# mllam/neural-lam

Measured on AMD Instinct MI355X. Metric: training sample-steps/s (on_after_batch_transfer+fwd+wmse+bwd+allreduce+AdamW), GraphCast-LAM, MEPS-shaped grid, higher is better.
Workload: dtype f32; 1 GPU; cfg2: graph_lam, grid 238x268 (63784 nodes), 17 state vars, hidden_dim 64, 4 processor layers, ar_steps 1, batch 1/GPU, g2m/m2m/m2g edges 79236/57616/255136; global_batch=1, parallelism=dp1

## Files before the change

### include/nlam_hip.h

```cpp
#ifndef NLAM_HIP_H
#define NLAM_HIP_H

#include <stdint.h>

#ifdef __cplusplus
extern "C" {
#endif

#define NLAM_ABI_VERSION 8
#define NLAM_MAX_SRC 3
#define NLAM_MAX_CAT 6

#define NLAM_EINVAL (-1)
#define NLAM_EUNSUP (-2)

#define NLAM_F_ADD_SRC0   1u
#define NLAM_F_ADD_SRC1   2u
#define NLAM_F_MEAN       4u
#define NLAM_F_SILU_B     8u
#define NLAM_F_PRE_ADD   16u
#define NLAM_F_LEAF_WGRAD 32u
#define NLAM_F_WPACK_READY 64u
#define NLAM_F_NO_ACT 128u
#define NLAM_F_STORE_BF16 (1u << 10)
// ... 190 lines not shown
int64_t nlam_mlp_bwd_gemm_workspace_floats(const nlam_mlp_bwd_t* p);
int32_t nlam_mlp_bwd_gemm_blocks(const nlam_mlp_bwd_t* p);
int32_t nlam_mlp_fwd_gemm(const nlam_mlp_fwd_t* p, void* hip_stream);
int32_t nlam_mlp_bwd_gemm(const nlam_mlp_bwd_t* p, void* hip_stream);

typedef struct {
    const float* W1;
    const float* W2;
    float* fwd_image;
    float* bwd_image;
    int32_t hid, dout, nsrc;
    int32_t ldw1;
    int32_t width[NLAM_MAX_SRC];
    uint32_t flags;
} nlam_pack_job_t;
int64_t nlam_mlp_pack_floats(const nlam_pack_job_t* job, int32_t which);
typedef struct {
    unsigned char bytes[64];
} nlam_pack_rec_t;
int32_t nlam_mlp_fwd_pack_records(const nlam_mlp_fwd_t* p, nlam_pack_rec_t* out, int32_t cap, int32_t* kind);
int32_t nlam_mlp_bwd_pack_records(const nlam_mlp_bwd_t* p, nlam_pack_rec_t* out, int32_t cap, int32_t* kind);
int32_t nlam_pack_records(const nlam_pack_rec_t* recs_device, int32_t n, int32_t kind, void* hip_stream);
int32_t nlam_mlp_pack(const nlam_pack_job_t* jobs_device, int32_t njobs, void* hip_stream);

#define NLAM_MAX_GROUP 8
int32_t nlam_mlp_group_blocks(const int64_t* tiles, int32_t n, int32_t* blocks);
int32_t nlam_mlp_fwd_group(const nlam_mlp_fwd_t* ps, int32_t n, void* hip_stream);
int32_t nlam_mlp_bwd_group(const nlam_mlp_bwd_t* ps, int32_t n, void* hip_stream);
int32_t nlam_mlp_fwd_family(const nlam_mlp_fwd_t* p);
int32_t nlam_mlp_bwd_family(const nlam_mlp_bwd_t* p);
int32_t nlam_mlp_bwd_group_blocks(const nlam_mlp_bwd_t* ps, int32_t n, int32_t* blocks);
int32_t nlam_wgrad(const nlam_wgrad_t* p, void* hip_stream);
int32_t nlam_wgrad_group(const nlam_wgrad_t* ps, int32_t n, void* hip_stream);

int32_t nlam_segment_sum_groups(int64_t in_bstride, int32_t nseg, int32_t width);
int32_t nlam_segment_sum(const float* in, int64_t in_bstride, const int32_t* ptr, const int32_t* order,
                         const float* scale, float* out, int32_t nseg, int32_t width, int32_t batch,
                         void* hip_stream);
int32_t nlam_segment_sum_acc(const float* in, int64_t in_bstride, const int32_t* ptr, const int32_t* order,
                         const float* scale, float* out, int32_t nseg, int32_t width, int32_t batch,
                         void* hip_stream);
int32_t nlam_segment_sum_add(const float* in, int64_t in_bstride, const int32_t* ptr, const int32_t* order, const float* scale,
                             const float* extra, float* out, int32_t nseg, int32_t width, int32_t batch, void* hip_stream);

int32_t nlam_segment_sum_bf16(const uint16_t* in, int64_t in_bstride, const int32_t* ptr, const int32_t* order,
                              const float* scale, float* out, int32_t nseg, int32_t width, int32_t batch, void* hip_stream);

int32_t nlam_split_combine(float* buf, int64_t bstride, const int32_t* ptr, const int32_t* src, const int32_t* dst, int32_t n,
                           int32_t width, int32_t batch, void* hip_stream);

int32_t nlam_reduce_partials(const float* partials, int32_t nparts, int64_t stride, int32_t n, float* out,
                             int32_t accumulate, void* hip_stream);

#define NLAM_MAX_REDUCE_JOBS 40
typedef struct {
    const float* partials;
    float* out;
    int64_t stride;
    int32_t nparts;
    int32_t n;
    int32_t accumulate;
    int32_t ncols;
    int32_t ld;
    int32_t _pad;
} nlam_reduce_job_t;
typedef struct {
// ... 410 lines not shown
```

### neural_lam_amd/_lib.py

```python
from __future__ import annotations

import ctypes as C
import os
from pathlib import Path

HERE = Path(__file__).resolve().parent
LIB_PATH = Path(os.environ["NLAM_LIB"]) if os.environ.get("NLAM_LIB") else HERE / "libnlam_hip.so"

NLAM_MAX_SRC = 3
NLAM_MAX_CAT = 6
NLAM_MAX_REDUCE_JOBS = 40
NLAM_MAX_GROUP = 8
F_ADD_SRC0, F_ADD_SRC1, F_MEAN, F_SILU_B, F_PRE_ADD, F_LEAF_WGRAD, F_WPACK_READY, F_NO_ACT = 1, 2, 4, 8, 16, 32, 64, 128
F_STORE_BF16, F_A_BF16, F_S_BF16 = 1 << 10, 1 << 10, 1 << 11
F_ACC_DSRC0 = 1 << 12
F_WGRAD_SOLO = 1 << 13
TUNE_WBF_MIN_SUPERTILES = 1
TUNE_WGRAD_CHUNKS = 2
TUNE_LIN_WGS = 3
TUNE_WGRAD_MIN_PARTS = 4
TUNE_WGRAD_BIG_MIN_ROWS = 5
TUNE_WBF_HALF = 6
TUNE_LIN_GEMM = 7
TUNE_WBF_V4 = 8
# ... 84 lines not shown
    "nlam_mlp_bwd",
    "nlam_mlp_fwd_gemm_workspace_floats",
    "nlam_mlp_bwd_gemm_workspace_floats",
    "nlam_mlp_bwd_gemm_blocks",
    "nlam_mlp_fwd_gemm",
    "nlam_mlp_bwd_gemm",
    "nlam_mlp_pack_floats",
    "nlam_mlp_pack",
    "nlam_mlp_fwd_pack_records",
    "nlam_mlp_bwd_pack_records",
    "nlam_pack_records",
    "nlam_wgrad",
    "nlam_segment_sum",
    "nlam_segment_sum_acc",
    "nlam_segment_sum_add",
    "nlam_split_combine",
    "nlam_segment_sum_bf16",
    "nlam_store_bf16_supported",
    "nlam_reduce_partials",
    "nlam_reduce_jobs",
    "nlam_reduce_jobs_waves",
    "nlam_wmse_fwd",
    "nlam_wmse_bwd",
    "nlam_adamw_step",
    "nlam_adamw_step_resident",
    "nlam_standardize",
    "nlam_mlp_group_blocks",
    "nlam_mlp_fwd_group",
    "nlam_mlp_bwd_group",
    "nlam_mlp_fwd_family",
    "nlam_mlp_bwd_family",
    "nlam_mlp_bwd_group_blocks",
    "nlam_wgrad_group",
    "nlam_linear",
    "nlam_linear_plan",
    "nlam_segment_sum_groups",
    "nlam_pre_add_supported",
    "nlam_step_tail_fwd",
    "nlam_step_tail_bwd",
    "nlam_loss_fwd",
    "nlam_loss_bwd",
    "nlam_step_tail_loss_fwd",
    "nlam_step_tail_loss_bwd",
    "nlam_step_tail_ext_fwd",
    "nlam_step_tail_ext_bwd",
    "nlam_eval_metrics",
    "nlam_eval_workspace_floats",
    "nlam_concat",
    "nlam_window_len",
    "nlam_window_batch",
    "nlam_window_batch_ens",
    "nlam_window_moments",
    "nlam_moments_workspace_doubles",
    "nlam_grad_sumsq_workspace_doubles",
    "nlam_grad_sumsq",
    "nlam_adamw_step_controlled",
    "nlam_accum_begin",
    "nlam_adamw_step_accum",
    "nlam_adamw_step_resident_ema",
    "nlam_adamw_step_controlled_ema",
    "nlam_flat_swap",
    "nlam_forecast_init",
    "nlam_forecast_head",
    "nlam_forecast_tail",
    "nlam_forecast_finish",
    "nlam_forecast_workspace_floats",
# ... 672 lines not shown
    lib.nlam_window_moments.restype = i32
    lib.nlam_moments_workspace_doubles.argtypes = [i32, i32, i64, i32]
    lib.nlam_moments_workspace_doubles.restype = i64
    lib.nlam_grad_sumsq_workspace_doubles.argtypes = [i64]
    lib.nlam_grad_sumsq_workspace_doubles.restype = i64
    lib.nlam_grad_sumsq.argtypes = [vp, i64, vp, i64, f32, vp, vp]
    lib.nlam_grad_sumsq.restype = i32
    lib.nlam_adamw_step_controlled.argtypes = [C.POINTER(OptCtl), vp]
    lib.nlam_adamw_step_controlled.restype = i32
    lib.nlam_accum_begin.argtypes = [vp, i64, vp, vp]
    lib.nlam_accum_begin.restype = i32
    lib.nlam_adamw_step_accum.argtypes = [C.POINTER(OptCtl), C.POINTER(Accum), vp]
    lib.nlam_adamw_step_accum.restype = i32
    lib.nlam_adamw_step_resident_ema.argtypes = [vp, vp, vp, vp, i64, f32, f32, f32, f32, f32, vp, vp, f32, vp, C.POINTER(Ema)]
    lib.nlam_adamw_step_resident_ema.restype = i32
    lib.nlam_adamw_step_controlled_ema.argtypes = [C.POINTER(OptCtl), C.POINTER(Accum), C.POINTER(Ema), vp]
    lib.nlam_adamw_step_controlled_ema.restype = i32
    lib.nlam_flat_swap.argtypes = [vp, vp, i64, vp]
    lib.nlam_flat_swap.restype = i32
    lib.nlam_mlp_group_blocks.argtypes = [C.POINTER(C.c_int64), i32, C.POINTER(C.c_int32)]
    lib.nlam_mlp_group_blocks.restype = i32
    lib.nlam_mlp_fwd_group.argtypes = [C.POINTER(MlpFwd), i32, vp]
    lib.nlam_mlp_fwd_group.restype = i32
    lib.nlam_mlp_bwd_group.argtypes = [C.POINTER(MlpBwd), i32, vp]
    lib.nlam_mlp_bwd_group.restype = i32
    lib.nlam_mlp_fwd_family.argtypes = [C.POINTER(MlpFwd)]
    lib.nlam_mlp_fwd_family.restype = i32
    lib.nlam_mlp_bwd_family.argtypes = [C.POINTER(MlpBwd)]
    lib.nlam_mlp_bwd_family.restype = i32
    lib.nlam_mlp_bwd_group_blocks.argtypes = [C.POINTER(MlpBwd), i32, C.POINTER(i32)]
    lib.nlam_mlp_bwd_group_blocks.restype = i32
    lib.nlam_wgrad_group.argtypes = [C.POINTER(Wgrad), i32, vp]
    lib.nlam_wgrad_group.restype = i32
    lib.nlam_pre_add_supported.argtypes = [C.POINTER(MlpFwd)]
    lib.nlam_pre_add_supported.restype = i32
    lib.nlam_linear.argtypes = [C.POINTER(Linear), vp]
    lib.nlam_linear.restype = i32
    lib.nlam_linear_plan.argtypes = [C.POINTER(Linear)]
    lib.nlam_linear_plan.restype = i32
    lib.nlam_segment_sum_groups.argtypes = [i64, i32, i32]
    lib.nlam_segment_sum_groups.restype = i32
    lib.nlam_standardize.argtypes = [C.POINTER(StdJobs), vp]
    lib.nlam_standardize.restype = i32
    if lib.nlam_abi_version() != ABI_VERSION:
        raise RuntimeError("libnlam_hip.so ABI version mismatch")
    if os.environ.get("NLAM_LIN_WGS"):
        lib.nlam_set_tuning(TUNE_LIN_WGS, int(os.environ["NLAM_LIN_WGS"]))
    if os.environ.get("NLAM_WGRAD_BIG_MIN_ROWS"):
        lib.nlam_set_tuning(TUNE_WGRAD_BIG_MIN_ROWS, int(os.environ["NLAM_WGRAD_BIG_MIN_ROWS"]))
    if os.environ.get("NLAM_WGRAD_MIN_PARTS"):
        lib.nlam_set_tuning(TUNE_WGRAD_MIN_PARTS, int(os.environ["NLAM_WGRAD_MIN_PARTS"]))
    if os.environ.get("NLAM_WBF_HALF"):
        check(lib.nlam_set_tuning(TUNE_WBF_HALF, int(os.environ["NLAM_WBF_HALF"])), "nlam_set_tuning(NLAM_WBF_HALF)")
    if os.environ.get("NLAM_WBF_V4"):
        lib.nlam_set_tuning(TUNE_WBF_V4, int(os.environ["NLAM_WBF_V4"]))
    if os.environ.get("NLAM_LIN_GEMM"):
        lib.nlam_set_tuning(TUNE_LIN_GEMM, int(os.environ["NLAM_LIN_GEMM"]))
    if os.environ.get("NLAM_WGRAD_LDMA"):
        check(lib.nlam_set_tuning(TUNE_WGRAD_LDMA, int(os.environ["NLAM_WGRAD_LDMA"])), "nlam_set_tuning(NLAM_WGRAD_LDMA)")
    if os.environ.get("NLAM_WBF_EDGE"):
        check(lib.nlam_set_tuning(TUNE_WBF_EDGE, int(os.environ["NLAM_WBF_EDGE"])), "nlam_set_tuning(NLAM_WBF_EDGE)")
    if os.environ.get("NLAM_WGRAD_LDMA_VAR"):
        check(lib.nlam_set_tuning(TUNE_WGRAD_LDMA_VAR, int(os.environ["NLAM_WGRAD_LDMA_VAR"])), "nlam_set_tuning(NLAM_WGRAD_LDMA_VAR)")
    if os.environ.get("NLAM_WGRAD_DMA_R"):
        check(lib.nlam_set_tuning(TUNE_WGRAD_DMA_R, int(os.environ["NLAM_WGRAD_DMA_R"])), "nlam_set_tuning(NLAM_WGRAD_DMA_R)")
    if os.environ.get("NLAM_CHAIN_CUS"):
# ... 75 lines not shown
```

### neural_lam_amd/csrc/nlam_hip.hip

```cpp

#include <hip/hip_runtime.h>
#include <stdint.h>
#include <type_traits>

#include "../../include/nlam_hip.h"
#include <dlfcn.h>
#include <stdlib.h>
#include <string.h>

#ifndef NLAM_TU
#define NLAM_TU 0
#endif
#ifndef NLAM_RES_PRE
#define NLAM_RES_PRE 3
#endif
#ifndef NLAM_BWD_G_BATCH
#define NLAM_BWD_G_BATCH 2
#endif
#ifndef NLAM_LW_PREFETCH_X
#define NLAM_LW_PREFETCH_X 1
#endif
#ifndef NLAM_BWD_Z_EARLY
#define NLAM_BWD_Z_EARLY 1
#endif
#ifndef NLAM_BWD_R_EARLY
#define NLAM_BWD_R_EARLY 0
#endif
#ifndef NLAM_LIN_SK
#define NLAM_LIN_SK 4
#endif
#define NLAM_IN_TU(k) (NLAM_TU == 0 || NLAM_TU == (k))

namespace nlam_detail {
int32_t fwd_narrow(const nlam_mlp_fwd_t* p, hipStream_t stream);
int32_t bwd_narrow(const nlam_mlp_bwd_t* p, hipStream_t stream);
int32_t wgrad_narrow(const nlam_wgrad_t* p, int plan, hipStream_t stream);
int32_t fwd_wide(const nlam_mlp_fwd_t* p, int plan, hipStream_t stream);
int32_t bwd_wide(const nlam_mlp_bwd_t* p, int plan, hipStream_t stream);
int32_t fwd_wide_group(const nlam_mlp_fwd_t* ps, int n, hipStream_t stream);
int32_t bwd_wide_group(const nlam_mlp_bwd_t* ps, int n, hipStream_t stream);
int32_t fwd_check(const nlam_mlp_fwd_t* p);
int32_t bwd_check(const nlam_mlp_bwd_t* p);
int32_t wgrad_wide(const nlam_wgrad_t* p, hipStream_t stream);
int32_t fwd_wbf(const nlam_mlp_fwd_t* p, int plan, hipStream_t stream);
int32_t bwd_wbf(const nlam_mlp_bwd_t* p, int plan, hipStream_t stream);
int32_t wgrad_wbf(const nlam_wgrad_t* p, int plan, hipStream_t stream);
int32_t wgrad_wbf_group(const nlam_wgrad_t* ps, int n, hipStream_t stream);
extern int wbf_min_supertiles;
extern int wbf_half;
extern int wbf_v4;
extern int wgrad_chunks_per_wg;
extern int wgrad_ldma;
extern int chain_cus;
extern int wgrad_max_wgs;
extern int wbf_edge;
extern int wgrad_ldma_var;
extern int wgrad_dma_r;
extern int wgrad_min_parts;
extern int wgrad_min_parts_wide;
extern int wgrad_big_min_rows;
extern int lin_resident_wgs;
extern int lin_gemm;
extern long lin_gemm_big_rows;
}

typedef float f32x4 __attribute__((ext_vector_type(4)));
typedef float f32x16 __attribute__((ext_vector_type(16)));

#define MFMA32(a, b, c) __builtin_amdgcn_mfma_f32_32x32x2f32((a), (b), (c), 0, 0, 0)
// ... 2214 lines not shown
                p.vec_partials[((size_t)wg_id * kVecRows + 4 + wave) * p.vec_stride + lane] = s;
            }
        }
    }
}

template <int HB, int OB, int NS, bool RO = false>
__global__ __launch_bounds__(kBlockThreads) void mlp_bwd_fast_kernel(const nlam_mlp_bwd_t p) {
    mlp_bwd_fast_body<HB, OB, NS, false, kWavesPerBlock, RO>(p, xcd_slot((int)blockIdx.x, (int)gridDim.x), (int)gridDim.x);
}

struct bwd_group_t {
    nlam_mlp_bwd_t g[NLAM_MAX_GROUP];
    int n;
    int first[NLAM_MAX_GROUP + 1];
};

constexpr int kLeafWaves = 4;
template <int HB, int OB, int NS, bool LW>
__global__ __launch_bounds__(LW ? kLeafWaves * 64 : kBlockThreads) void mlp_bwd_fast_group_kernel(const bwd_group_t G) {
    int gi = 0;
#pragma unroll
    for (int k = 1; k < NLAM_MAX_GROUP; ++k)
        if (k < G.n && (int)blockIdx.x >= G.first[k]) gi = k;
    mlp_bwd_fast_body<HB, OB, NS, LW, LW ? kLeafWaves : kWavesPerBlock>(G.g[gi], (int)blockIdx.x - G.first[gi], G.first[gi + 1] - G.first[gi]);
}

constexpr int kWgradThreads = 256;
constexpr int kWgradRows = 32;
constexpr int kWgTile = kWgradRows * 64;


template <int NBW, bool SILU, int NS, int R>
__global__ __launch_bounds__(kWgradThreads) void wgrad_dma_kernel(const nlam_wgrad_t p) {
    static_assert(NS >= 0 && NS <= NLAM_MAX_SRC && R >= 1 && (NS > 0 || R == 1), "run-time source count: one chunk per interval");
    constexpr int MS = NS > 0 ? NS : NLAM_MAX_SRC;
    extern __shared__ __attribute__((aligned(16))) float smem[];
    const int nsrc = NS > 0 ? NS : p.nsrc;
    const int ntile = 1 + nsrc;
    const int lane = threadIdx.x & 63;
    const int wave = __builtin_amdgcn_readfirstlane(threadIdx.x >> 6);
    const int i = lane & 31, hi = lane >> 5;
    const int MB = (p.m + 31) >> 5;

    int blk_mb[NBW], blk_tile[NBW], blk_nb[NBW], blk_col0[NBW], blk_w[NBW];
    {
        int nb_total = 0;
#pragma unroll
        for (int s = 0; s < MS; ++s)
            if (s < nsrc) nb_total += (p.src[s].width + 31) >> 5;
#pragma unroll
        for (int q = 0; q < NBW; ++q) {
            const int blk = wave + 4 * q;
            blk_mb[q] = -1;
            blk_tile[q] = 1;
            blk_nb[q] = 0;
            blk_col0[q] = 0;
            blk_w[q] = 0;
            if (blk < MB * nb_total) {
                blk_mb[q] = blk / nb_total;
                int nbg = blk % nb_total, off = 0;
                bool found = false;
#pragma unroll
                for (int s = 0; s < MS; ++s) {
                    if (s >= nsrc || found) continue;
                    const int nbs = (p.src[s].width + 31) >> 5;
                    if (nbg < nbs) {
// ... 16 lines not shown
    for (int q = 0; q < NBW; ++q)
#pragma unroll
        for (int r = 0; r < 16; ++r) acc[q][r] = 0.f;

    const int cpb = (p.rows + kWgradRows - 1) / kWgradRows;
    const long total_chunks = (long)cpb * p.batch;
    const int lrow = lane >> 4, lcol = (lane & 15) << 2;

    typedef unsigned long long u64;
    const char* const abase = reinterpret_cast<const char*>(p.A + lcol);
    const bool acol = lcol < p.m;
    const int arows = p.rows;
    const unsigned apitch = (unsigned)p.m * 4u;
    const long abatch = (long)p.rows * p.m * 4;
    const char* sbase[MS];
    const int* sidx[MS];
    long sbatch[MS];
    unsigned spitch[MS];
    bool scol[MS];
#pragma unroll
    for (int s = 0; s < MS; ++s) {
        const bool on = s < nsrc;
        sbase[s] = on ? reinterpret_cast<const char*>(p.src[s].ptr + lcol) : nullptr;
        sidx[s] = on ? p.src[s].idx : nullptr;
        sbatch[s] = on ? (long)p.src[s].bstride * 4 : 0;
        spitch[s] = on ? (unsigned)p.src[s].width * 4u : 0u;
        scol[s] = on && lcol < p.src[s].width;
    }
    const char* zero16 = reinterpret_cast<const char*>(g_zero16);
    asm volatile("" : "+s"(zero16));
    const int trow = wave * 8 + lrow;
    float* const lds_row = smem + (size_t)(wave * 8) * 64;

    const int g = (int)gridDim.x, c0 = xcd_slot((int)blockIdx.x, g);
    const int nseq = c0 < total_chunks ? (int)((total_chunks - c0 + g - 1) / g) : 0;
    const int gq = g / cpb, gr = g % cpb;
    struct Cursor {
        int b, c;
    };
    auto advance = [&](Cursor& k) {
        k.b += gq;
        k.c += gr;
        if (k.c >= cpb) {
            k.c -= cpb;
            ++k.b;
        }
    };
    Cursor kl = {c0 / cpb, c0 % cpb};
    Cursor ki = kl;

    auto load_idx = [&](int(&ix)[2][MS], int(&pr)[2]) {
        const int r0 = kl.c * kWgradRows;
        const int nr = min(kWgradRows, arows - r0);
#pragma unroll
        for (int gi = 0; gi < 2; ++gi) {
            const int r = trow + 4 * gi;
            const bool rv = r < nr;
            const int prow = r0 + (rv ? r : 0);
            pr[gi] = rv ? prow : -1;
#pragma unroll
            for (int s = 0; s < MS; ++s) {
                int v = prow;
                if (rv && sidx[s] != nullptr) v = sidx[s][prow];
                ix[gi][s] = rv ? v : -1;
            }
        }
        advance(kl);
// ... 43 lines not shown
        __syncthreads();
#pragma unroll
        for (int j = 0; j < R; ++j)
            if (k0 + R + j < nseq) issue(lds_row + (buf ^ 1) * stage_floats + j * ntile * kWgTile, ix[j], pr[j]);
#pragma unroll
        for (int j = 0; j < R; ++j)
            if (k0 + 2 * R + j < nseq) load_idx(ix[j], pr[j]);
#pragma unroll
        for (int j = 0; j < R; ++j) {
            if (k0 + j >= nseq) continue;
            const float* At = smem + (size_t)buf * stage_floats + (size_t)(j * ntile) * kWgTile;
#pragma unroll
            for (int q = 0; q < NBW; ++q) {
                if (blk_mb[q] >= 0) {
                    const float* Bt = At + (size_t)blk_tile[q] * kWgTile;
                    const int ac = blk_mb[q] * 32 + i, bc = blk_nb[q] * 32 + i;
                    float a[kWgradRows / 2], bv[kWgradRows / 2];
#pragma unroll
                    for (int ks = 0; ks < kWgradRows / 2; ++ks) {
                        a[ks] = At[(2 * ks + hi) * 64 + ac];
                        bv[ks] = Bt[(2 * ks + hi) * 64 + bc];
                    }
                    if constexpr (SILU) {
#pragma unroll
                        for (int ks = 0; ks < kWgradRows / 2; ++ks) bv[ks] = silu_f(bv[ks]);
                    }
#pragma unroll
                    for (int ks = 0; ks < kWgradRows / 2; ++ks) acc[q] = MFMA32(a[ks], bv[ks], acc[q]);
                }
            }
        }
        buf ^= 1;
    }
    float* P = p.partials + (size_t)blockIdx.x * p.m * p.n;
#pragma unroll
    for (int q = 0; q < NBW; ++q) {
        if (blk_mb[q] >= 0) {
            const int n = blk_col0[q] + i;
#pragma unroll
            for (int r = 0; r < 16; ++r) {
                const int m = blk_mb[q] * 32 + (r & 3) + 8 * (r >> 2) + 4 * hi;
                if (m < p.m && n < blk_w[q]) P[(size_t)m * p.n + n] = acc[q][r];
            }
        }
    }
}

template <int NBW>
__global__ __launch_bounds__(kWgradThreads) void wgrad_kernel(const nlam_wgrad_t p) {
    extern __shared__ __attribute__((aligned(16))) float smem[];
    const int MP = round_up(p.m, 32), NP = round_up(p.n, 32);
    const int SA = MP + 4, SB = NP + 4;
    float* As = smem;
    float* Bs = As + kWgradRows * SA;
    const int NB = NP / 32;
    const int nblocks = (MP / 32) * NB;
    const int lane = threadIdx.x & 63, wave = threadIdx.x >> 6;
    const int i = lane & 31, hi = lane >> 5;

    f32x16 acc[NBW];
#pragma unroll
    for (int q = 0; q < NBW; ++q)
#pragma unroll
        for (int r = 0; r < 16; ++r) acc[q][r] = 0.f;

    for (int s = threadIdx.x; s < kWgradRows * (SA + SB); s += blockDim.x) smem[s] = 0.f;
    __syncthreads();

    const int chunks_per_batch = (p.rows + kWgradRows - 1) / kWgradRows;
    const long total_chunks = (long)chunks_per_batch * p.batch;
    for (long ch = blockIdx.x; ch < total_chunks; ch += gridDim.x) {
        const int b = (int)(ch / chunks_per_batch);
        const int r0 = (int)(ch % chunks_per_batch) * kWgradRows;
        const int nr = min(kWgradRows, p.rows - r0);
        for (int s = threadIdx.x; s < kWgradRows * p.m; s += blockDim.x) {
            const int r = s / p.m, c = s % p.m;
            As[r * SA + c] = (r < nr) ? p.A[((size_t)b * p.rows + r0 + r) * p.m + c] : 0.f;
        }
// ... 2214 lines not shown
    for (int s = 0; s < p->nsrc; ++s)
        if ((reinterpret_cast<uintptr_t>(p->src[s].ptr) & 15) != 0 || ((p->src[s].bstride * sesz) & 15) != 0) return false;
    return true;
}

int wgrad_plan_of(const nlam_wgrad_t* p, int ldma) {
    if (p == nullptr || p->A == nullptr || p->partials == nullptr || p->nsrc < 1 || p->nsrc > NLAM_MAX_SRC) return NLAM_EINVAL;
    int n = 0;
    for (int s = 0; s < p->nsrc; ++s) n += p->src[s].width;
    if (n != p->n || p->m < 1 || p->nparts < 1) return NLAM_EINVAL;
    const bool abf = (p->flags & NLAM_F_A_BF16) != 0, sbf = (p->flags & NLAM_F_S_BF16) != 0;
    if (wgrad_is_smalln(p)) return abf || sbf ? NLAM_EUNSUP : NLAM_WGP_SMALLN;
    if (!wgrad_is_wide(p)) {
        if (abf || sbf) return NLAM_EUNSUP;
        return wgrad_is_narrow_dma(p) && wgrad_dma_aligned(p, 4) ? NLAM_WGP_DMA : NLAM_WGP_NARROW;
    }
    const int wns = wgrad_wbf_ns(p);
    if (wns == 0) return abf || sbf ? NLAM_EUNSUP : NLAM_WGP_WIDE;
    const bool big = wgrad_wbf_big(p), silu = (p->flags & NLAM_F_SILU_B) != 0;
    if (abf || sbf) {
        if (wns != 1 || !abf || (sbf && (p->nsrc != 1 || p->src[0].idx != nullptr || !silu)) || (!sbf && silu)) return NLAM_EUNSUP;
        if ((reinterpret_cast<uintptr_t>(p->A) & 3) != 0 ||
            (sbf && ((reinterpret_cast<uintptr_t>(p->src[0].ptr) & 3) != 0 || (p->src[0].bstride & 1) != 0)))
            return NLAM_EINVAL;
        if (big && (ldma & 1) && p->m % 8 == 0 && (!sbf || p->src[0].width % 8 == 0) && wgrad_dma_aligned(p, sbf ? 2 : 4))
            return NLAM_WGP_LDMA_B;
        return big ? NLAM_WGP_WBF_B_BIG : NLAM_WGP_WBF_B;
    }
    if (big && ((wns == 1 && (ldma & 2)) || (wns == 3 && (ldma & 4))) && wgrad_dma_aligned(p, 4))
        return wns == 1 ? NLAM_WGP_LDMA_1 : NLAM_WGP_LDMA_3;
    return big ? NLAM_WGP_WBF_BIG : NLAM_WGP_WBF;
}

void group_blocks(const long* tiles, int n, int* blocks) {
    long tot = 0;
    for (int k = 0; k < n; ++k) tot += tiles[k] < 1 ? 1 : tiles[k];
    for (int k = 0; k < n; ++k) {
        const long t = tiles[k] < 1 ? 1 : tiles[k];
        long b = tot <= kMaxGridBlocks ? t : (t * kMaxGridBlocks) / tot;
        if (b < 1) b = 1;
        if (b > t) b = t;
        blocks[k] = (int)b;
    }
}

template <typename G>
void group_prefix(G& grp, int n, const int* count) {
    grp.n = n;
    grp.first[0] = 0;
    for (int k = 0; k < n; ++k) grp.first[k + 1] = grp.first[k] + count[k];
    for (int k = n + 1; k <= NLAM_MAX_GROUP; ++k) grp.first[k] = grp.first[n];
}

bool same_fwd_shape(const nlam_mlp_fwd_t& a, const nlam_mlp_fwd_t& b) {
    if (a.hid != b.hid || a.dout != b.dout || a.ncat != b.ncat) return false;
    return (a.flags & ~NLAM_F_WPACK_READY) == (b.flags & ~NLAM_F_WPACK_READY) && (a.ln_w == nullptr) == (b.ln_w == nullptr);
}
bool same_bwd_shape(const nlam_mlp_bwd_t& a, const nlam_mlp_bwd_t& b) {
    if (a.hid != b.hid || a.dout != b.dout) return false;
    const WideCfg ca = wide_cfg(bwd_wide_maxw(&a)), cb = wide_cfg(bwd_wide_maxw(&b));
    if (ca.nwv != cb.nwv || ca.fb != cb.fb) return false;
    return (a.flags & ~NLAM_F_WPACK_READY) == (b.flags & ~NLAM_F_WPACK_READY) && (a.ln_w == nullptr) == (b.ln_w == nullptr);
}

void wide_group_blocks(const long* tiles, int n, long cap, int* blocks) {
    long tot = 0;
// ... 1028 lines not shown
    hipStream_t stream = (hipStream_t)hip_stream;
    switch (plan) {
    case NLAM_WGP_SMALLN:
    case NLAM_WGP_DMA:
    case NLAM_WGP_NARROW: return nlam_detail::wgrad_narrow(p, plan, stream);
    case NLAM_WGP_WIDE: return nlam_detail::wgrad_wide(p, stream);
    case NLAM_WGP_WBF:
    case NLAM_WGP_WBF_BIG:
    case NLAM_WGP_WBF_B:
    case NLAM_WGP_WBF_B_BIG:
    case NLAM_WGP_LDMA_B:
    case NLAM_WGP_LDMA_1:
    case NLAM_WGP_LDMA_3: return nlam_detail::wgrad_wbf(p, plan, stream);
    default: return plan < 0 ? plan : NLAM_EINVAL;
    }
}

int32_t nlam_wgrad_group(const nlam_wgrad_t* ps, int32_t n, void* hip_stream) {
    NLAM_RANGE("nlam_wgrad_group");
    if (ps == nullptr || n < 1 || n > NLAM_MAX_GROUP) return NLAM_EINVAL;
    const int plan0 = wgrad_plan_of(&ps[0], 0);
    for (int k = 0; k < n; ++k) {
        const nlam_wgrad_t* p = &ps[k];
        const int plan = wgrad_plan_of(p, 0);
        if (plan == NLAM_EINVAL || p->nparts != nlam_wgrad_nparts(p)) return NLAM_EINVAL;
        if ((plan != NLAM_WGP_WBF && plan != NLAM_WGP_WBF_BIG) || plan != plan0) return NLAM_EUNSUP;
        if (p->m != ps[0].m || p->n != ps[0].n || p->nsrc != ps[0].nsrc || p->flags != ps[0].flags) return NLAM_EUNSUP;
        for (int s = 0; s < p->nsrc; ++s)
            if (p->src[s].width != ps[0].src[s].width) return NLAM_EUNSUP;
    }
    return nlam_detail::wgrad_wbf_group(ps, n, (hipStream_t)hip_stream);
}

}
#endif

#if NLAM_IN_TU(4)
namespace {
template <int NS, bool SILU, bool ABF, bool SBFS>
int32_t launch_wgrad_wbf(bool big, dim3 grid, size_t lds, hipStream_t stream, const nlam_wgrad_t& p) {
    if (big) return launch<wgrad_wbf_kernel<NS, SILU, 1, 4, 2, 4, ABF, SBFS>>(grid, dim3(4 * 2 * 64), lds, stream, p);
    return launch<wgrad_wbf_kernel<NS, SILU, 1, 2, 2, 2, ABF, SBFS>>(grid, dim3(2 * 2 * 64), lds, stream, p);
}
template <int NS, bool ABF, bool SBF, bool SILU, int R, int NB>
int32_t launch_wgrad_ldma(dim3 grid, hipStream_t stream, const nlam_wgrad_t& p) {
    return launch<wgrad_ldma_kernel<NS, ABF, SBF, SILU, R, NB>>(grid, dim3(512), WgLdma<ABF, SBF, SILU, R, NB>::LDS, stream, p);
}
}

int32_t nlam_detail::wgrad_wbf(const nlam_wgrad_t* p, int plan, hipStream_t stream) {
    const int wns = wgrad_wbf_ns(p);
    const bool big = plan != NLAM_WGP_WBF && plan != NLAM_WGP_WBF_B;
    const int winm = big ? 256 : 128, winn = big ? 256 : 128;
    const size_t lds = (size_t)2 * ((winm + winn) / 32) * wns * 1024;
    const dim3 grid(p->nparts, wgrad_windows_of(p, winm, winn));
    const bool silu = (p->flags & NLAM_F_SILU_B) != 0;
    const bool sb = (p->flags & NLAM_F_S_BF16) != 0;
    const int var = nlam_detail::wgrad_ldma_var;
    switch (plan) {
    case NLAM_WGP_LDMA_B:
        if (sb) {
            if (var == 1) return launch_wgrad_ldma<1, true, true, true, 32, 5>(grid, stream, *p);
            if (var == 2) return launch_wgrad_ldma<1, true, true, true, 16, 6>(grid, stream, *p);
            if (var == 3) return launch_wgrad_ldma<1, true, true, true, 16, 8>(grid, stream, *p);
            return launch_wgrad_ldma<1, true, true, true, 32, 4>(grid, stream, *p);
        }
// ... 79 lines not shown
    for (int s = 0; s < p->nsrc; ++s) nb_total += (p->src[s].width + 31) / 32;
    if (plan == NLAM_WGP_DMA) {
        const int nblocks = ((p->m + 31) / 32) * nb_total;
        const int nbw = (nblocks + 3) / 4;
        const bool silu = (p->flags & NLAM_F_SILU_B) != 0;
        if (nbw == p->nsrc && (!silu || p->nsrc == 1)) {
            int r = nlam_detail::wgrad_dma_r > 0 ? nlam_detail::wgrad_dma_r : kWgradDmaR[p->nsrc - 1];
            if (p->nsrc > 1 && r > 2) r = 2;
            if (p->nsrc == 1)
                return pick<1, 2, 4>(r, [&](auto rr) {
                    return pick_bool(silu, [&](auto sl) { return launch_wgrad_dma<1, sl, 1, rr>(stream, *p); });
                });
            return pick<1, 2>(r, [&](auto rr) {
                if (p->nsrc == 2) return launch_wgrad_dma<2, false, 2, rr>(stream, *p);
                return launch_wgrad_dma<3, false, 3, rr>(stream, *p);
            });
        }
        const size_t lds = (size_t)2 * (1 + p->nsrc) * kWgTile * sizeof(float);
        return pick<1, 2, 3>(nbw < 1 ? 1 : nbw, [&](auto nb) {
            return pick_bool(silu, [&](auto sl) {
                return launch<wgrad_dma_kernel<nb, sl, 0, 1>>(dim3(p->nparts), dim3(kWgradThreads), lds, stream, *p);
            });
        });
    }
    const int MP = (p->m + 31) / 32 * 32, NP = (p->n + 31) / 32 * 32;
    const int nblocks = (MP / 32) * (NP / 32);
    const size_t lds = (size_t)kWgradRows * (MP + 4 + NP + 4) * sizeof(float);
    const int nbw = (nblocks + 3) / 4;
    const int ywin = (nblocks + 11) / 12;
    const dim3 grid(p->nparts, nbw > 3 ? ywin : 1);
    return pick<1, 2, 3>(nbw < 1 ? 1 : (nbw > 3 ? 3 : nbw), [&](auto nb) {
        return launch<wgrad_kernel<nb>>(grid, dim3(kWgradThreads), lds, stream, *p);
    });
}
#endif

#if NLAM_IN_TU(5)
extern "C" {

int64_t nlam_window_len(int64_t n_state_times, int64_t n_forcing_times, int32_t ar_steps, int32_t past, int32_t future) {
    const int64_t window = (int64_t)(past > 2 ? past : 2) + ar_steps + future;
    int64_t n = n_state_times - window + 1;
    if (n_forcing_times >= 0 && n_forcing_times - window + 1 < n) n = n_forcing_times - window + 1;
    return n > 0 ? n : 0;
}

int32_t nlam_window_batch(const nlam_window_t* p, void* hip_stream) {
    NLAM_RANGE("nlam_window_batch");
    if (p == nullptr || p->state == nullptr || p->sample_idx == nullptr || p->init_states == nullptr || p->target_states == nullptr)
        return NLAM_EINVAL;
    if (p->batch < 0 || p->nodes < 0 || p->d_state < 1 || p->d_forcing < 0 || p->ar_steps < 1 || p->ar_steps > 256 ||
        p->num_past_forcing_steps < 0 || p->num_future_forcing_steps < 0 || p->n_times < 1)
        return NLAM_EINVAL;
    if (p->d_forcing > 0 && (p->forcing == nullptr || p->forcing_windowed == nullptr)) return NLAM_EINVAL;
    if ((p->state_mean == nullptr) != (p->state_std == nullptr) || (p->forcing_mean == nullptr) != (p->forcing_std == nullptr)) return NLAM_EINVAL;
    if (p->state_mean != nullptr && p->d_forcing > 0 && p->forcing_mean == nullptr) return NLAM_EINVAL;
    if (nlam_window_len(p->n_times, p->d_forcing > 0 ? p->n_times : -1, p->ar_steps, p->num_past_forcing_steps, p->num_future_forcing_steps) < 1)
        return NLAM_EINVAL;
    if (p->batch == 0 || p->nodes == 0) return 0;
    const long window = p->num_past_forcing_steps + p->num_future_forcing_steps + 1;
    const long e_state = (long)p->nodes * p->d_state;
    const long e_forc = (long)p->nodes * p->d_forcing * window;
    if (e_state >= (1L << 31) || e_forc >= (1L << 31) || p->batch > 65535) return NLAM_EUNSUP;
    long blocks = ((e_state > e_forc ? e_state : e_forc) + 2047) / 2048;
    if (blocks < 1) blocks = 1;
    if (blocks > 512) blocks = 512;
// ... 718 lines not shown
```

### neural_lam_amd/ops.py

```python
from __future__ import annotations

import contextlib
import ctypes as C
import math
import os
from dataclasses import dataclass, field

import torch

from . import _lib as L


def _vec_stride(hid: int, dout: int) -> int:
    return max(64, (max(hid, dout) + 63) // 64 * 64)



_MM_FLAGS = {"f32": 0, "bf16": 1 << 8, "bf16x2": 2 << 8, "bf16x3": 3 << 8}
MATMUL_MODE = os.environ.get("NLAM_MATMUL", "bf16x3")


def set_matmul_mode(mode: str, bwd: str | None = None):
    global MATMUL_MODE, MATMUL_MODE_BWD
    if mode not in _MM_FLAGS or (bwd is not None and bwd not in ("bf16x2", "bf16x3")):
# ... 229 lines not shown
    if prev == "auto":
        WGRAD_SOLO_MODE = mode
    try:
        yield
    finally:
        WGRAD_SOLO_MODE = prev


def _wgrad_solo() -> int:
    if WGRAD_SOLO_MODE != "auto":
        return L.F_WGRAD_SOLO if WGRAD_SOLO_MODE == "1" else 0
    return 0 if (OVERLAP.active or PROFILE.enabled) else L.F_WGRAD_SOLO


class _WgradOverlap:

    NSTREAMS = int(os.environ.get("NLAM_WGRAD_STREAMS", "4"))

    def __init__(self):
        self.streams = []
        self.assigned = {}
        self.active = False
        self.capturing = False
        self.keep = []

    def begin(self, deferred=None):
        if not self.streams:
            self.streams = list(stream_layout()["sides"]) if QUEUE_SIDES != "0" else [torch.cuda.Stream() for _ in range(max(1, self.NSTREAMS))]
        self.active = True
        self.assigned = {}
        self.keep = []
        self.deferred = deferred
        self.capturing = torch.cuda.is_current_stream_capturing()

    deferred = None

    def index_for(self, owner):
        k = self.assigned.get(id(owner))
        if k is None:
            k = self.assigned[id(owner)] = len(self.assigned) % len(self.streams)
        return k

    def stream_for(self, owner):
        return self.streams[self.index_for(owner)]

    def hold(self, side, *tensors):
        for t in tensors:
            if t is None:
                continue
            if self.capturing:
                self.keep.append(t)
            else:
                t.record_stream(side)

    def run(self, owner, hold, fn, dead_end=False):
        if self.deferred is not None:
            self.keep.extend(t for t in hold if t is not None)
            self.deferred.fork(self.index_for(owner), fn, dead_end)
            return
        side = self.stream_for(owner)
        side.wait_stream(torch.cuda.current_stream())
        self.hold(side, *hold)
        with torch.cuda.stream(side):
            fn()

    def end(self):
        if self.deferred is not None:
            d, self.deferred = self.deferred, None
            try:
                d.finish()
            finally:
                self.keep = []
                self.active = False
            return
        if self.active:
            for st in self.streams:
                torch.cuda.current_stream().wait_stream(st)
        self.keep = []
        self.active = False


OVERLAP = _WgradOverlap()


class WeightPacker:

    def __init__(self):
        self.enabled = os.environ.get("NLAM_PACK_WEIGHTS", "1") == "1"
        self.entries = {}
        self.table = None
        self.table_entries = []
        self.dirty = False
        self.step_id = 0
        self.wide_enabled = os.environ.get("NLAM_PACK_WIDE", "1") == "1"
        self.wide = {}
        self.wide_tables = {}
        self.wide_dirty = False
        self._retired = []

# ... 274 lines not shown
        direct = _direct_grad(param, shape)
        if out is None:
            out = param.grad if direct else (torch.zeros if ncols else torch.empty)(tuple(shape), device=self.dev, dtype=torch.float32)
        self.keep.append(out)
        self.reserve(1)
        j = self.jobs.job[self.jobs.njobs]
        j.partials, j.out, j.stride, j.nparts, j.accumulate = partials_ptr, out.data_ptr() + 4 * out_off, stride, nparts, 1 if direct else 0
        j.n, j.ncols, j.ld = (shape[0] * ncols, ncols, shape[1]) if ncols else (math.prod(shape), 0, 0)
        self.jobs.njobs += 1
        return out, direct

    def flush(self):
        if self.jobs.njobs > 0:
            L.check(L.load().nlam_reduce_jobs(C.byref(self.jobs), _stream()), "nlam_reduce_jobs")
            self.jobs.njobs = 0


def _mlp_reduce_jobs(batch, part1, part2, vecp, nblk, vs, vec_rows, dims, params, needs, has_ln, ncols=0):
    hid, kin, dout = dims
    res = [None] * 6
    mat = lambda part: (_ptr(part), part.shape[0], part.shape[1] * part.shape[2])
    vec = lambda r: (vecp.data_ptr() + r * vs * 4, nblk, vec_rows * vs)
    jobs = ((part1 is not None and mat(part1), (hid, kin)), (needs[1] and vec(0), (hid,)), (part2 is not None and mat(part2), (dout, hid)),
            (needs[3] and vec(1), (dout,)), (has_ln and needs[4] and vec(2), (dout,)), (has_ln and needs[5] and vec(3), (dout,)))
    for slot, (job, shape) in enumerate(jobs):
        if job:
            out, direct = batch.add(*job, shape, params[slot], ncols=ncols if slot == 0 else 0)
            if not direct:
                res[slot] = out
    return res


def _wgrad_request(A, m, n, B, rows, src_list, flags, dev):
    q = L.Wgrad()
    q.A, q.m, q.batch, q.rows, q.nsrc, q.flags, q.n = _ptr(A), m, B, rows, len(src_list), flags, n
    for k, (t, bstride, w, idx) in enumerate(src_list):
        _fill_src(q.src[k], t, bstride, w, idx)
    nparts = L.load().nlam_wgrad_nparts(C.byref(q))
    partials = torch.empty((nparts, m, n), device=dev, dtype=torch.float32)
    q.partials, q.nparts = _ptr(partials), nparts
    return q, partials


@dataclass
class _WgradItem:

    B: int
    rows: int
    hid: int
    dout: int
    kin: int
    mm_flags: int
    dz1: torch.Tensor
    dz2: torch.Tensor
    z1: torch.Tensor
    vecp: torch.Tensor
    nblk: int
    vs: int
    src_list: list
    params: tuple
    needs: list
    has_ln: bool


def _wide_wpack(p, nwp, side, key, dev, use_packer=True):
    wbuf = PACKER.get_wide(side, p, nwp, key) if (PACKER is not None and use_packer) else None
    if wbuf is not None:
        p.wpack, p.wpack_floats, p.flags = wbuf.data_ptr(), nwp, int(p.flags) | L.F_WPACK_READY
        return None
    wpack = torch.empty((nwp,), device=dev, dtype=torch.float32)
    p.wpack, p.wpack_floats = _ptr(wpack), nwp
    return wpack


# ... 349 lines not shown
        q, partials = _wgrad_request(A, m, n, B, rows, src_list, flags | ctx.mm_flags | _wgrad_solo(), dev)
        key = ("wgrad", rows * B, m, n)

        def wg_meta():
            nsrc_b = sum(t.shape[-2] * w * t.element_size() * (B if bstride != 0 or B == 1 else 1) for (t, bstride, w, idx) in src_list)
            nbytes = A.numel() * A.element_size() + partials.numel() * 4 + nsrc_b
            nmin = A.numel() * A.element_size() + nsrc_b + m * n * 4
            narrow = m <= 64 and all(w <= 64 for (_, _, w, _) in src_list)
            name, mf = ("f32", 0) if narrow else _mm_executed(ctx.mm_flags, m, m, [w for (_, _, w, _) in src_list])
            return {"flops": 2.0 * rows * B * m * n, "bytes": float(nbytes), "bytes_min": float(nmin), "mm": name, "mfmas_per_block": mf,
                    "what": "weight gradient dW = A^T [gathered B], rows = MFMA K"}

        L.check(PROFILE.launch(key, lambda: lib.nlam_wgrad(C.byref(q), _stream()), wg_meta), "nlam_wgrad")
        return partials

    src_list = []
    for k in range(1 if pre else nsrc):
        b_, bstride = ctx.binfo[k]
        src_list.append((bases[k], bstride if b_ == B or B == 1 else 0, widths[k], geom.src_idx[k]))
    kin1 = widths[0] if pre else kin
    results = [None] * 6

    def launch_weights():
        part1 = wgrad(dz1, hid, src_list, kin1, L.F_A_BF16 if sbf else 0) if needs[1] else None
        part2 = wgrad(dz2, dpad, [(z1, rows * hid, hid, None)], hid, L.F_SILU_B | ((L.F_A_BF16 | L.F_S_BF16) if sbf else 0)) if needs[3] else None
        batch = _ReduceBatch(dev)
        results[:] = _mlp_reduce_jobs(batch, part1, part2, vecp, nblk, vs, 4, (hid, kin, dout), prm, pneeds, ctx.has_ln, ncols=kin1 if pre else 0)
        batch.flush()
        if on_side:
            OVERLAP.hold(torch.cuda.current_stream(), part1, part2)
        if GRAD_LISTENER is not None:
            GRAD_LISTENER.note_done([q for q, nd in zip(prm, pneeds) if nd and q is not None and _direct_grad(q, q.shape)])

    if whole_side:
        OVERLAP.run(prm[0], (g_out, g_aggr, xhat, rstd, wpack, dz1, dz2, vecp, z1, *bases), lambda: (launch_data(), launch_weights()), dead_end=True)
    elif on_side:
        OVERLAP.run(prm[0], (dz1, dz2, vecp, z1, *bases), launch_weights)
    else:
        launch_weights()
    dW1, db1, dW2, db2, dg, dbt = results

    if isinstance(acc_report, torch.Tensor):
        dsrc[0] = acc_report if dsrc[0] is None else dsrc[0].add_(acc_report)
    grads_src = [None if g is None else _unbatch_grad(g, ctx.src_shapes[k], B) for k, g in enumerate(dsrc)]
    return (None, dW1, db1, dW2, db2, dg, dbt, *grads_src)


@dataclass
class ChunkedGeometry:

    nsrc: int
    chunks: list
    rows: int
    src_mode: list
    src_idx: list
    flags_fwd: int = 0
    flags_bwd: int = 0
    rowptr: torch.Tensor | None = None
    perm: torch.Tensor | None = None
    inv_deg: torch.Tensor | None = None
    seg_of_row: torch.Tensor | None = None
    num_rec: int = 0
    mean: bool = False
    scatter: list = field(default_factory=lambda: [None, None, None])


def _row_window(x: torch.Tensor):
    t, B, bstride, _ = as_batched(x)
    return t, B, bstride

# ... 1505 lines not shown
```

Baseline: 607.6 sample-steps/s.

## Batch small MLP weight-gradient kernels into one grouped DMA launch

```diff
diff --git a/include/nlam_hip.h b/include/nlam_hip.h
--- a/include/nlam_hip.h
+++ b/include/nlam_hip.h
@@ -246,6 +246,8 @@
 int32_t nlam_mlp_bwd_group_blocks(const nlam_mlp_bwd_t* ps, int32_t n, int32_t* blocks);
 int32_t nlam_wgrad(const nlam_wgrad_t* p, void* hip_stream);
 int32_t nlam_wgrad_group(const nlam_wgrad_t* ps, int32_t n, void* hip_stream);
+int32_t nlam_wgrad_dma_group_supported(const nlam_wgrad_t* p);
+int32_t nlam_wgrad_dma_group(const nlam_wgrad_t* ps, int32_t n, void* hip_stream);
 
 int32_t nlam_segment_sum_groups(int64_t in_bstride, int32_t nseg, int32_t width);
 int32_t nlam_segment_sum(const float* in, int64_t in_bstride, const int32_t* ptr, const int32_t* order,
diff --git a/neural_lam_amd/_lib.py b/neural_lam_amd/_lib.py
--- a/neural_lam_amd/_lib.py
+++ b/neural_lam_amd/_lib.py
@@ -140,6 +140,8 @@
     "nlam_mlp_bwd_family",
     "nlam_mlp_bwd_group_blocks",
     "nlam_wgrad_group",
+    "nlam_wgrad_dma_group",
+    "nlam_wgrad_dma_group_supported",
     "nlam_linear",
     "nlam_linear_plan",
     "nlam_segment_sum_groups",
@@ -878,6 +880,10 @@
     lib.nlam_mlp_bwd_group_blocks.restype = i32
     lib.nlam_wgrad_group.argtypes = [C.POINTER(Wgrad), i32, vp]
     lib.nlam_wgrad_group.restype = i32
+    lib.nlam_wgrad_dma_group.argtypes = [C.POINTER(Wgrad), i32, vp]
+    lib.nlam_wgrad_dma_group.restype = i32
+    lib.nlam_wgrad_dma_group_supported.argtypes = [C.POINTER(Wgrad)]
+    lib.nlam_wgrad_dma_group_supported.restype = i32
     lib.nlam_pre_add_supported.argtypes = [C.POINTER(MlpFwd)]
     lib.nlam_pre_add_supported.restype = i32
     lib.nlam_linear.argtypes = [C.POINTER(Linear), vp]
diff --git a/neural_lam_amd/csrc/nlam_hip.hip b/neural_lam_amd/csrc/nlam_hip.hip
--- a/neural_lam_amd/csrc/nlam_hip.hip
+++ b/neural_lam_amd/csrc/nlam_hip.hip
@@ -35,6 +35,7 @@
 int32_t fwd_narrow(const nlam_mlp_fwd_t* p, hipStream_t stream);
 int32_t bwd_narrow(const nlam_mlp_bwd_t* p, hipStream_t stream);
 int32_t wgrad_narrow(const nlam_wgrad_t* p, int plan, hipStream_t stream);
+int32_t wgrad_dma_group(const nlam_wgrad_t* ps, int n, hipStream_t stream);
 int32_t fwd_wide(const nlam_mlp_fwd_t* p, int plan, hipStream_t stream);
 int32_t bwd_wide(const nlam_mlp_bwd_t* p, int plan, hipStream_t stream);
 int32_t fwd_wide_group(const nlam_mlp_fwd_t* ps, int n, hipStream_t stream);
@@ -2315,7 +2316,7 @@
 
 
 template <int NBW, bool SILU, int NS, int R>
-__global__ __launch_bounds__(kWgradThreads) void wgrad_dma_kernel(const nlam_wgrad_t p) {
+__device__ __forceinline__ void wgrad_dma_body(const nlam_wgrad_t& p, const int wg_id, const int wg_count) {
     static_assert(NS >= 0 && NS <= NLAM_MAX_SRC && R >= 1 && (NS > 0 || R == 1), "run-time source count: one chunk per interval");
     constexpr int MS = NS > 0 ? NS : NLAM_MAX_SRC;
     extern __shared__ __attribute__((aligned(16))) float smem[];
@@ -2398,7 +2399,7 @@
     const int trow = wave * 8 + lrow;
     float* const lds_row = smem + (size_t)(wave * 8) * 64;
 
-    const int g = (int)gridDim.x, c0 = xcd_slot((int)blockIdx.x, g);
+    const int g = wg_count, c0 = xcd_slot(wg_id, g);
     const int nseq = c0 < total_chunks ? (int)((total_chunks - c0 + g - 1) / g) : 0;
     const int gq = g / cpb, gr = g % cpb;
     struct Cursor {
@@ -2508,7 +2509,7 @@
         }
         buf ^= 1;
     }
-    float* P = p.partials + (size_t)blockIdx.x * p.m * p.n;
+    float* P = p.partials + (size_t)wg_id * p.m * p.n;
 #pragma unroll
     for (int q = 0; q < NBW; ++q) {
         if (blk_mb[q] >= 0) {
@@ -2520,6 +2521,26 @@
             }
         }
     }
+}
+
+template <int NBW, bool SILU, int NS, int R>
+__global__ __launch_bounds__(kWgradThreads) void wgrad_dma_kernel(const nlam_wgrad_t p) {
+    wgrad_dma_body<NBW, SILU, NS, R>(p, (int)blockIdx.x, (int)gridDim.x);
+}
+
+struct wgrad_dma_group_t {
+    nlam_wgrad_t g[NLAM_MAX_GROUP];
+    int n;
+    int first[NLAM_MAX_GROUP + 1];
+};
+static_assert(sizeof(wgrad_dma_group_t) <= 4096, "wgrad_dma_group_t is passed by value: it must fit the kernel-argument segment");
+template <int NBW, bool SILU, int NS, int R>
+__global__ __launch_bounds__(kWgradThreads) void wgrad_dma_group_kernel(const wgrad_dma_group_t G) {
+    int gi = 0;
+#pragma unroll
+    for (int k = 1; k < NLAM_MAX_GROUP; ++k)
+        if (k < G.n && (int)blockIdx.x >= G.first[k]) gi = k;
+    wgrad_dma_body<NBW, SILU, NS, R>(G.g[gi], (int)blockIdx.x - G.first[gi], G.first[gi + 1] - G.first[gi]);
 }
 
 template <int NBW>
@@ -4800,6 +4821,20 @@
     return big ? NLAM_WGP_WBF_BIG : NLAM_WGP_WBF;
 }
 
+int wgrad_dma_group_ns(const nlam_wgrad_t* p) {
+    if (p == nullptr || p->nsrc < 1 || p->nsrc > NLAM_MAX_SRC || p->m < 1) return 0;
+    if ((p->flags & (NLAM_F_A_BF16 | NLAM_F_S_BF16)) != 0) return 0;
+    int n = 0, nb_total = 0;
+    for (int s = 0; s < p->nsrc; ++s) {
+        n += p->src[s].width;
+        nb_total += (p->src[s].width + 31) / 32;
+    }
+    if (n != p->n || wgrad_is_smalln(p) || wgrad_is_wide(p) || !wgrad_is_narrow_dma(p)) return 0;
+    const int nbw = (((p->m + 31) / 32) * nb_total + 3) / 4;
+    const bool silu = (p->flags & NLAM_F_SILU_B) != 0;
+    return nbw == p->nsrc && (!silu || p->nsrc == 1) ? p->nsrc : 0;
+}
+
 void group_blocks(const long* tiles, int n, int* blocks) {
     long tot = 0;
     for (int k = 0; k < n; ++k) tot += tiles[k] < 1 ? 1 : tiles[k];
@@ -5894,6 +5929,28 @@
     return nlam_detail::wgrad_wbf_group(ps, n, (hipStream_t)hip_stream);
 }
 
+int32_t nlam_wgrad_dma_group_supported(const nlam_wgrad_t* p) { return wgrad_dma_group_ns(p) > 0 ? 1 : 0; }
+
+int32_t nlam_wgrad_dma_group(const nlam_wgrad_t* ps, int32_t n, void* hip_stream) {
+    NLAM_RANGE("nlam_wgrad_dma_group");
+    if (ps == nullptr || n < 1 || n > NLAM_MAX_GROUP) return NLAM_EINVAL;
+    for (int k = 0; k < n; ++k) {
+        const nlam_wgrad_t* p = &ps[k];
+        if (wgrad_plan_of(p, nlam_detail::wgrad_ldma) == NLAM_EINVAL || p->batch < 1 || p->rows < 1) return NLAM_EINVAL;
+        if (p->nparts != nlam_wgrad_nparts(p)) return NLAM_EINVAL;
+        for (int s = 0; s < p->nsrc; ++s)
+            if (p->src[s].ptr == nullptr) return NLAM_EINVAL;
+    }
+    for (int k = 0; k < n; ++k) {
+        const nlam_wgrad_t* p = &ps[k];
+        if (wgrad_plan_of(p, nlam_detail::wgrad_ldma) != NLAM_WGP_DMA || wgrad_dma_group_ns(p) == 0) return NLAM_EUNSUP;
+        if (p->m != ps[0].m || p->n != ps[0].n || p->nsrc != ps[0].nsrc || p->flags != ps[0].flags) return NLAM_EUNSUP;
+        for (int s = 0; s < p->nsrc; ++s)
+            if (p->src[s].width != ps[0].src[s].width) return NLAM_EUNSUP;
+    }
+    return nlam_detail::wgrad_dma_group(ps, n, (hipStream_t)hip_stream);
+}
+
 }
 #endif
 
@@ -6039,6 +6096,25 @@
     return pick<1, 2, 3>(nbw < 1 ? 1 : (nbw > 3 ? 3 : nbw), [&](auto nb) {
         return launch<wgrad_kernel<nb>>(grid, dim3(kWgradThreads), lds, stream, *p);
     });
+}
+
+int32_t nlam_detail::wgrad_dma_group(const nlam_wgrad_t* ps, int n, hipStream_t stream) {
+    wgrad_dma_group_t G;
+    int parts[NLAM_MAX_GROUP];
+    for (int k = 0; k < n; ++k) {
+        G.g[k] = ps[k];
+        parts[k] = ps[k].nparts;
+    }
+    for (int k = n; k < NLAM_MAX_GROUP; ++k) G.g[k] = ps[0];
+    group_prefix(G, n, parts);
+    const int ns = ps[0].nsrc;
+    const dim3 grid(G.first[n]), block(kWgradThreads);
+    const size_t lds = (size_t)2 * (1 + ns) * kWgTile * sizeof(float);
+    if (ns == 1)
+        return pick_bool((ps[0].flags & NLAM_F_SILU_B) != 0,
+                         [&](auto sl) { return launch<wgrad_dma_group_kernel<1, sl, 1, 1>>(grid, block, lds, stream, G); });
+    if (ns == 2) return launch<wgrad_dma_group_kernel<2, false, 2, 1>>(grid, block, lds, stream, G);
+    return launch<wgrad_dma_group_kernel<3, false, 3, 1>>(grid, block, lds, stream, G);
 }
 #endif
 
diff --git a/neural_lam_amd/ops.py b/neural_lam_amd/ops.py
--- a/neural_lam_amd/ops.py
+++ b/neural_lam_amd/ops.py
@@ -285,6 +285,7 @@
         self.keep = []
         self.deferred = deferred
         self.capturing = torch.cuda.is_current_stream_capturing()
+        WGRAD_BATCH.reset()
 
     deferred = None
 
@@ -318,6 +319,13 @@
             fn()
 
     def end(self):
+        if self.active:
+            try:
+                WGRAD_BATCH.flush()
+            except BaseException:
+                self.deferred, self.keep, self.active = None, [], False
+                raise
+        WGRAD_BATCH.reset()
         if self.deferred is not None:
             d, self.deferred = self.deferred, None
             try:
@@ -658,14 +666,145 @@
 
 
 def _wgrad_request(A, m, n, B, rows, src_list, flags, dev):
+    q, nparts = _wgrad_describe(A, m, n, B, rows, src_list, flags)
+    partials = torch.empty((nparts, m, n), device=dev, dtype=torch.float32)
+    q.partials, q.nparts = _ptr(partials), nparts
+    return q, partials
+
+
+def _wgrad_describe(A, m, n, B, rows, src_list, flags):
     q = L.Wgrad()
     q.A, q.m, q.batch, q.rows, q.nsrc, q.flags, q.n = _ptr(A), m, B, rows, len(src_list), flags, n
     for k, (t, bstride, w, idx) in enumerate(src_list):
         _fill_src(q.src[k], t, bstride, w, idx)
-    nparts = L.load().nlam_wgrad_nparts(C.byref(q))
-    partials = torch.empty((nparts, m, n), device=dev, dtype=torch.float32)
-    q.partials, q.nparts = _ptr(partials), nparts
-    return q, partials
+    return q, L.load().nlam_wgrad_nparts(C.byref(q))
+
+
+
+WGRAD_BATCH_K = int(os.environ.get("NLAM_WGRAD_BATCH", "5"))
+WGRAD_BATCH_CHUNKS = int(os.environ.get("NLAM_WGRAD_BATCH_CHUNKS", "2"))
+
+
+def wgrad_is_small(rows: int, batch: int, nparts: int, chunks_per_wg: int | None = None) -> bool:
+    per = WGRAD_BATCH_CHUNKS if chunks_per_wg is None else chunks_per_wg
+    return batch * ((rows + 31) // 32) <= per * nparts
+
+
+def wgrad_batch_policy(pending_owners, pending_jobs: int, owner, njobs: int, k: int, cap: int | None = None, max_jobs: int | None = None):
+    cap = L.NLAM_MAX_GROUP if cap is None else cap
+    max_jobs = L.NLAM_MAX_REDUCE_JOBS if max_jobs is None else max_jobs
+    before = len(pending_owners) > 0 and (owner in pending_owners or len(pending_owners) + 1 > cap or pending_jobs + njobs > max_jobs)
+    waiting = (0 if before else len(pending_owners)) + 1
+    return before, waiting >= min(max(k, 1), cap)
+
+
+@dataclass
+class _WgradMember:
+
+    owner: object
+    B: int
+    rows: int
+    dims: tuple
+    req1: tuple
+    req2: tuple
+    vecp: torch.Tensor
+    nblk: int
+    vs: int
+    params: tuple
+    needs: list
+    has_ln: bool
+    ncols: int
+    njobs: int
+
+    def tensors(self):
+        out = [self.vecp]
+        for A, _m, _n, src_list, _f in (self.req1, self.req2):
+            out.append(A)
+            out.extend(t for (t, _b, _w, _i) in src_list if isinstance(t, torch.Tensor))
+        return out
+
+
+class _WgradBatch:
+
+    def __init__(self):
+        self.members = []
+        self.seen = set()
+
+    def reset(self):
+        self.members, self.seen = [], set()
+
+    def enabled(self) -> bool:
+        return WGRAD_BATCH_K > 0 and WGRAD_BATCH_CHUNKS > 0
+
+    def wants(self, B, rows, req1, req2) -> bool:
+        lib = L.load()
+        for A, m, n, src_list, flags in (req1, req2):
+            q, nparts = _wgrad_describe(A, m, n, B, rows, src_list, flags)
+            if not lib.nlam_wgrad_dma_group_supported(C.byref(q)) or not wgrad_is_small(rows, B, nparts):
+                return False
+        return True
+
+    def add(self, mem: _WgradMember):
+        before, after = wgrad_batch_policy({id(m.owner) for m in self.members}, sum(m.njobs for m in self.members), id(mem.owner), mem.njobs, WGRAD_BATCH_K)
+        if before:
+            self.flush()
+        self.members.append(mem)
+        self.seen.add(id(mem.owner))
+        if after:
+            self.flush()
+
+    def flush(self):
+        members, self.members = self.members, []
+        if members:
+            OVERLAP.run(self, tuple(t for m in members for t in m.tensors()), lambda: _wgrad_batch_launch(members))
+
+
+WGRAD_BATCH = _WgradBatch()
+
+
+def _wgrad_batch_launch(members):
+    lib = L.load()
+    dev = members[0].vecp.device
+    parts, classes = [], {}
+    for mem in members:
+        got = []
+        for A, m, n, src_list, flags in (mem.req1, mem.req2):
+            q, partials = _wgrad_request(A, m, n, mem.B, mem.rows, src_list, flags, dev)
+            key = (m, n, flags, tuple(w for (_t, _b, w, _i) in src_list))
+            classes.setdefault(key, []).append((q, A, src_list, partials))
+            got.append(partials)
+        parts.append(got)
+    for (m, n, _flags, _widths), reqs in classes.items():
+        for g0 in range(0, len(reqs), L.NLAM_MAX_GROUP):
+            grp = reqs[g0 : g0 + L.NLAM_MAX_GROUP]
+            rc = -2
+            if len(grp) > 1:
+                arr = (L.Wgrad * len(grp))(*[r[0] for r in grp])
+                rows_all = sum(int(r[0].rows) * int(r[0].batch) for r in grp)
+
+                def meta(grp=grp, rows_all=rows_all, m=m, n=n):
+                    nbytes = sum(A.numel() * 4 + p_.numel() * 4 + sum(t.shape[-2] * w * 4 for (t, _b, w, _i) in sl if isinstance(t, torch.Tensor))
+                                 for (_q, A, sl, p_) in grp)
+                    return {"flops": 2.0 * rows_all * m * n, "bytes": float(nbytes), "bytes_min": float(nbytes - sum(r[3].numel() * 4 for r in grp) + len(grp) * m * n * 4),
+                            "mm": "f32", "mfmas_per_block": 0, "what": "weight gradients dW = A^T [gathered B] of several small MLPs in one grid"}
+
+                rc = PROFILE.launch(("wgrad_dma_group", rows_all, len(grp), m, n), lambda: lib.nlam_wgrad_dma_group(arr, len(grp), _stream()), meta)
+            if rc == -2:
+                for r in grp:
+                    L.check(PROFILE.launch(("wgrad", int(r[0].rows) * int(r[0].batch), m, n), lambda r=r: lib.nlam_wgrad(C.byref(r[0]), _stream())), "nlam_wgrad")
+            else:
+                L.check(rc, "nlam_wgrad_dma_group")
+    batch = _ReduceBatch(dev)
+    done = []
+    for mem, (part1, part2) in zip(members, parts):
+        batch.reserve(mem.njobs)
+        _mlp_reduce_jobs(batch, part1, part2, mem.vecp, mem.nblk, mem.vs, 4, mem.dims, mem.params, mem.needs, mem.has_ln, ncols=mem.ncols)
+        done.append([q for q, nd in zip(mem.params, mem.needs) if nd and q is not None and _direct_grad(q, q.shape)])
+    batch.flush()
+    OVERLAP.hold(torch.cuda.current_stream(), *[p_ for got in parts for p_ in got])
+    if GRAD_LISTENER is not None:
+        for d in done:
+            GRAD_LISTENER.note_done(d)
 
 
 @dataclass
@@ -1081,10 +1220,25 @@
         if GRAD_LISTENER is not None:
             GRAD_LISTENER.note_done([q for q, nd in zip(prm, pneeds) if nd and q is not None and _direct_grad(q, q.shape)])
 
-    if whole_side:
-        OVERLAP.run(prm[0], (g_out, g_aggr, xhat, rstd, wpack, dz1, dz2, vecp, z1, *bases), lambda: (launch_data(), launch_weights()), dead_end=True)
+    side_owner, handed_over = prm[0], False
+    if on_side and WGRAD_BATCH.enabled():
+        req1 = (dz1, hid, kin1, src_list, ctx.mm_flags | _wgrad_solo())
+        req2 = (dz2, dpad, hid, [(z1, rows * hid, hid, None)], L.F_SILU_B | ctx.mm_flags | _wgrad_solo())
+        if (not whole_side and not sbf and needs[1] and needs[3] and id(prm[0]) not in OVERLAP.assigned
+                and WGRAD_BATCH.wants(B, rows, req1, req2)):
+            njobs = 2 + sum(1 for x in (pneeds[1], pneeds[3], ctx.has_ln and pneeds[4], ctx.has_ln and pneeds[5]) if x)
+            WGRAD_BATCH.add(_WgradMember(prm[0], B, rows, (hid, kin, dout), req1, req2, vecp, nblk, vs, prm, pneeds, ctx.has_ln,
+                                         kin1 if pre else 0, njobs))
+            handed_over = True
+        elif id(prm[0]) in WGRAD_BATCH.seen:
+            WGRAD_BATCH.flush()
+            side_owner = WGRAD_BATCH
+    if handed_over:
+        pass
+    elif whole_side:
+        OVERLAP.run(side_owner, (g_out, g_aggr, xhat, rstd, wpack, dz1, dz2, vecp, z1, *bases), lambda: (launch_data(), launch_weights()), dead_end=True)
     elif on_side:
-        OVERLAP.run(prm[0], (dz1, dz2, vecp, z1, *bases), launch_weights)
+        OVERLAP.run(side_owner, (dz1, dz2, vecp, z1, *bases), launch_weights)
     else:
         launch_weights()
     dW1, db1, dW2, db2, dg, dbt = results
```

Result: faster. 614.7 sample-steps/s (median of 6 runs) (+1.2%).
